# JustinPrivitera/Real_Time_Ray_Tracer

Measured on AMD Instinct MI355X. Metric: Mrays/s + ms/frame at 3840x2160, 16 AO samples, 64 spheres; 1/2/4/8 GPU, higher is better.
Workload: dtype f32

## Files before the change

### include/rt/abi.h

```cpp
#ifndef RT_ABI_H
#define RT_ABI_H

#include <stddef.h>
#include <stdint.h>

#include "layout.h"

#ifdef __cplusplus
extern "C" {
#endif

#define RT_ABI_VERSION 1

enum {
  RT_OK = 0,
  RT_E_INVAL = -1,
  RT_E_NOMEM = -2,
  RT_E_HIP = -3,
  RT_E_NODEV = -4,
  RT_E_STATE = -5
};

enum {
  RT_PROG_AOP_COMPUTE = 1,
// ... 24 lines not shown
int rt_set_stream(rt_ctx* ctx, void* hip_stream);
int rt_use_own_stream(rt_ctx* ctx);
void* rt_get_stream(rt_ctx* ctx);
int rt_enable_pipelining(rt_ctx* ctx, int on, void* output_stream);
void* rt_get_output_stream(rt_ctx* ctx);
void* rt_image_stream(rt_ctx* ctx);
int rt_device_count(void);
int rt_synchronize(rt_ctx* ctx);
int rt_last_hip_error(rt_ctx* ctx);
int rt_debug_fail_next_event_query(rt_ctx* ctx, int hip_error);

int rt_upload_header(rt_ctx* ctx, const void* header, size_t bytes);
int rt_upload_rand_buffer(rt_ctx* ctx, const float* rand_vec4, size_t n_vec4);
int rt_run_program(rt_ctx* ctx, int program, int frame);
int rt_dispatch(rt_ctx* ctx, int mode, int frame);
int rt_compute_frames(rt_ctx* ctx, float* header, int mode, int frame, int n, uint64_t rand_seed,
                      int light_movement);
int rt_set_frame_batch(rt_ctx* ctx, int max_frames);
int rt_set_tile_schedule(rt_ctx* ctx, int on);
int rt_tile_schedule_state(rt_ctx* ctx);
int rt_tile_schedule_orders(rt_ctx* ctx);
int rt_set_cull_cache(rt_ctx* ctx, int on);
int rt_cull_cache_stats(rt_ctx* ctx, long long* fills, long long* cached_launches, size_t* table_bytes);
size_t rt_cull_key(const rt_config* cfg, const void* header, size_t header_bytes, void* key, size_t key_cap);
int rt_download(rt_ctx* ctx, float* pixels, float* normals, float* depth, float* image);
int rt_download_rect(rt_ctx* ctx, int x0, int x1, int y0, int y1, float* pixels, float* normals, float* depth,
                     float* image);
int rt_upload_gbuffer(rt_ctx* ctx, const float* pixels, const float* normals, const float* depth);
void* rt_image_device_ptr(rt_ctx* ctx);
int rt_bind_image(rt_ctx* ctx, void* device_ptr);

int rt_compute_one_shader(rt_ctx* ctx, void* ssbo, int frame_num, int program, float* image);
int rt_compute_two_shaders(rt_ctx* ctx, void* ssbo, int frame_num, int program1, int program2,
                           float* image);

typedef struct rt_group rt_group;
int rt_group_create(int n, const int* devices, const rt_config* cfg, const int* bounds, rt_group** out);
int rt_group_strip_copies(rt_group* g, int i);
int rt_group_force_copies(rt_group* g, int on);
int rt_group_destroy(rt_group* g);
int rt_group_size(rt_group* g);
int rt_group_bounds(rt_group* g, int* bounds);
int rt_group_set_bounds(rt_group* g, const int* bounds);
rt_ctx* rt_group_strip(rt_group* g, int i);
int rt_group_last_hip_error(rt_group* g);
int rt_group_enable_pipelining(rt_group* g, int on);
// ... 67 lines not shown
```

### real_time_ray_tracer_amd/_lib.py

```python
from __future__ import annotations

import ctypes as C
import os
from pathlib import Path

LIB_NAME = "librtrt.so"
LIB_PATH = Path(__file__).resolve().with_name(LIB_NAME)

RT_OK, RT_E_INVAL, RT_E_NOMEM, RT_E_HIP, RT_E_NODEV, RT_E_STATE = 0, -1, -2, -3, -4, -5
RT_PROG_AOP_COMPUTE = 1
RT_PROG_AOP_POSTPROCESSING = 2
RT_PROG_AO_COMPUTE = 3
RT_PROG_P_COMPUTE = 4
RT_PROG_H_COMPUTE = 5
RT_MODE_AO_PP, RT_MODE_AO, RT_MODE_PHONG, RT_MODE_PHONG_REFL = 1, 2, 3, 4
(RT_MATH_SIN, RT_MATH_RANDOM, RT_MATH_SQRT, RT_MATH_DIV, RT_MATH_NORMALIZE, RT_MATH_SPHERE, RT_MATH_SQRT_SWEEP,
 RT_MATH_RCP_SWEEP, RT_MATH_SQRT_TAIL_SWEEP, RT_MATH_SIN_RANGE, RT_MATH_SHADOW,
 RT_MATH_SIN_TABLE) = range(12)
RT_NUM_FRAMES = 8
RT_RECURSION_DEPTH = 20
RT_SHAPE_SPHERE, RT_SHAPE_RECTANGLE, RT_SHAPE_PLANE = 1, 3, 5
HDR_MODE, HDR_HORIZONTAL, HDR_VERTICAL, HDR_LLC, HDR_CAMERA, HDR_LIGHT, HDR_BACKGROUND = range(7)


# ... 10 lines not shown
SIGNATURES = {
    "rt_create": (C.c_int, [C.c_int, C.POINTER(rt_config), C.POINTER(_ctx)]),
    "rt_destroy": (C.c_int, [_ctx]),
    "rt_set_stream": (C.c_int, [_ctx, _vp]),
    "rt_use_own_stream": (C.c_int, [_ctx]),
    "rt_get_stream": (_vp, [_ctx]),
    "rt_enable_pipelining": (C.c_int, [_ctx, C.c_int, _vp]),
    "rt_get_output_stream": (_vp, [_ctx]),
    "rt_image_stream": (_vp, [_ctx]),
    "rt_device_count": (C.c_int, []),
    "rt_synchronize": (C.c_int, [_ctx]),
    "rt_last_hip_error": (C.c_int, [_ctx]),
    "rt_upload_header": (C.c_int, [_ctx, _vp, C.c_size_t]),
    "rt_upload_rand_buffer": (C.c_int, [_ctx, _fp, C.c_size_t]),
    "rt_run_program": (C.c_int, [_ctx, C.c_int, C.c_int]),
    "rt_dispatch": (C.c_int, [_ctx, C.c_int, C.c_int]),
    "rt_compute_frames": (C.c_int, [_ctx, _fp, C.c_int, C.c_int, C.c_int, C.c_uint64, C.c_int]),
    "rt_set_frame_batch": (C.c_int, [_ctx, C.c_int]),
    "rt_set_tile_schedule": (C.c_int, [_ctx, C.c_int]),
    "rt_tile_schedule_state": (C.c_int, [_ctx]),
    "rt_tile_schedule_orders": (C.c_int, [_ctx]),
    "rt_set_cull_cache": (C.c_int, [_ctx, C.c_int]),
    "rt_cull_cache_stats": (C.c_int, [_ctx, C.POINTER(C.c_longlong), C.POINTER(C.c_longlong), C.POINTER(C.c_size_t)]),
    "rt_cull_key": (C.c_size_t, [C.POINTER(rt_config), _vp, C.c_size_t, _vp, C.c_size_t]),
    "rt_download": (C.c_int, [_ctx, _fp, _fp, _fp, _fp]),
    "rt_download_rect": (C.c_int, [_ctx, C.c_int, C.c_int, C.c_int, C.c_int, _fp, _fp, _fp, _fp]),
    "rt_upload_gbuffer": (C.c_int, [_ctx, _fp, _fp, _fp]),
    "rt_image_device_ptr": (_vp, [_ctx]),
    "rt_bind_image": (C.c_int, [_ctx, _vp]),
    "rt_compute_one_shader": (C.c_int, [_ctx, _vp, C.c_int, C.c_int, _fp]),
    "rt_compute_two_shaders": (C.c_int, [_ctx, _vp, C.c_int, C.c_int, C.c_int, _fp]),
    "rt_group_create": (C.c_int, [C.c_int, C.POINTER(C.c_int), C.POINTER(rt_config), C.POINTER(C.c_int),
                                  C.POINTER(_grp)]),
    "rt_group_destroy": (C.c_int, [_grp]),
    "rt_group_size": (C.c_int, [_grp]),
    "rt_group_strip_copies": (C.c_int, [_grp, C.c_int]),
    "rt_group_force_copies": (C.c_int, [_grp, C.c_int]),
    "rt_group_bounds": (C.c_int, [_grp, C.POINTER(C.c_int)]),
    "rt_group_set_bounds": (C.c_int, [_grp, C.POINTER(C.c_int)]),
    "rt_group_strip": (_ctx, [_grp, C.c_int]),
    "rt_group_last_hip_error": (C.c_int, [_grp]),
    "rt_group_enable_pipelining": (C.c_int, [_grp, C.c_int]),
    "rt_group_bind_frame": (C.c_int, [_grp, _vp]),
    "rt_group_frame_device_ptr": (_vp, [_grp]),
    "rt_group_upload_header": (C.c_int, [_grp, _vp, C.c_size_t]),
    "rt_group_dispatch": (C.c_int, [_grp, C.c_int, C.c_int]),
# ... 90 lines not shown
```

### real_time_ray_tracer_amd/csrc/rt_kernels.h

```cpp
#pragma once
#include <hip/hip_runtime.h>

#ifndef RT_NRM_PLANES
#define RT_NRM_PLANES 1
#endif

namespace rt {

constexpr int kMaxFrames = 16;
constexpr int kMaxBatch = 32;
#ifndef RT_HY_BW
#define RT_HY_BW 2
#endif
constexpr int kHyBW = RT_HY_BW, kHyTile = 8 * RT_HY_BW;
constexpr int kCounters = 8;
constexpr int kCounterSlots = 256;

struct FrameParams {
  int W, H;
  int trace_row0, trace_rows;
  int band_row0, band_rows;
  int img_row0, img_rows;
  int nobj;
  int S;
  int spp, D, F, frame;
  int b1_min;
  int pool_rot;
  int tile_run;
  int post_sx, post_sy;
  float inv_spp, fW, fH;
  float inv_W, inv_H;
  float hx, hy, hz;
  float vx, vy, vz;
  float lx, ly, lz;
  float cx, cy, cz;
  float Lx, Ly, Lz;
  float4 bg;
  const float4* shapes;
  const float4* sph;
  const float4* planes;
  int nplanes;
  const float4* clus;
  const unsigned long long* clmask;
  const float4* camrel;
  int ncl;
  const float4* rb;
  float4* out_pix;
  float4* nrm;
  float4* dep;
  const float4* nrm_prev;
  const float4* dep_prev;
  float4* image;
  const float4* raw;
  const float4* hist_pix[kMaxFrames];
  const float4* hist_nrm[kMaxFrames];
  const float4* hist_dep[kMaxFrames];
  unsigned long long* counters;
  unsigned long long* row_counters;
  int mf_n, mf_slot0;
  float4 mf_light[kMaxBatch];
  const float4* mf_rb;
  const unsigned* tile_order;
  unsigned* tile_cost;
  const unsigned long long* cull;
};

constexpr int kAoPool = 256;
constexpr long long ao_pool_count(int trace_rows, int W, int spp) {
  const int TP = kAoPool / spp > 0 ? kAoPool / spp : 1;
  return ((long long)trace_rows * W + TP - 1) / TP;
}

constexpr int kMaxClusters = 64;
constexpr int kClusterWords = 4;

__host__ __device__ constexpr size_t sphere_table(int S) { return (size_t)4 * S; }
__host__ __device__ constexpr size_t plane_table(int S) { return (size_t)5 * S; }
__host__ __device__ constexpr size_t cluster_table(int S) { return (size_t)7 * S; }
__host__ __device__ constexpr size_t cluster_mask_table(int S) { return cluster_table(S) + kMaxClusters; }
__host__ __device__ constexpr size_t camrel_table(int S) {
  return cluster_mask_table(S) + (size_t)(1 + kMaxClusters) * kClusterWords / 2;
}
__host__ __device__ constexpr size_t rand_table(int S) { return camrel_table(S) + (size_t)S; }
__host__ __device__ constexpr size_t table_vec4(int S, int spp) { return rand_table(S) + (size_t)2 * spp; }

enum KernelId { K_AOP = 1, K_POST = 2, K_AO = 3, K_PHONG = 4, K_HYBRID = 5 };

hipError_t launch_program(int program, const FrameParams& p, hipStream_t stream);

hipError_t launch_cull_fill(const FrameParams& p, unsigned long long* table, hipStream_t stream);

struct GbufXfer {
  int W, R, r0, F, kind, to_ref;
  size_t n;
  float4* ref;
  float4* slot[kMaxFrames];
};
hipError_t launch_gbuf_convert(const GbufXfer& x, hipStream_t stream);

hipError_t launch_selftest(int fn, const float* d_in, float* d_out, size_t n, hipStream_t stream);

}
```

### real_time_ray_tracer_amd/csrc/rt_kernels_impl.h

```cpp
#pragma once
#include <hip/hip_runtime.h>

#include "rt_device.h"
#include "rt_kernels.h"

namespace rt {

namespace {

constexpr int kBlock = 256;
constexpr float kGamma = 1.0f / 2.2f;

__device__ __forceinline__ void stage_shapes(const FrameParams& P, float4* lds) {
  const int n = P.nobj;
  for (int k = threadIdx.x; k < 4 * n; k += blockDim.x) {
    int tab = k / n, i = k - tab * n;
    lds[k] = P.shapes[(size_t)tab * P.S + i];
  }
}

__device__ __forceinline__ f3 primary_dir(const FrameParams& P, float hp, float vp) {
  f3 a = mk(P.lx + hp * P.hx, P.ly + hp * P.hy, P.lz + hp * P.hz);
  return normalize(mk(a.x + vp * P.vx, a.y + vp * P.vy, a.z + vp * P.vz));
}
// ... 737 lines not shown

#ifndef RT_AO_MINW
#define RT_AO_MINW 7
#endif
constexpr int kAoMinWaves = RT_AO_MINW;
#ifndef RT_B1_SORT
#define RT_B1_SORT 1
#endif

struct AoConfig {
  static constexpr int SPPC = 0;
  static constexpr int DC = 0;
  static constexpr bool PL = false;
  static constexpr bool CLON = false;
  static constexpr bool CNT = true;
  static constexpr bool MF = false;
  static constexpr bool LAZY = true;
  static constexpr bool TAIL = false;
  static constexpr bool B1 = false;
  static constexpr bool PT = false;
  static constexpr bool PTW = false;
  static constexpr bool SORT = false;
  static constexpr bool CULLC = false;
  static constexpr int ABL = 0;
};
enum : unsigned {
  AO_PL = 1,
  AO_CLON = 2,
  AO_SORT = 4,
  AO_WIDE = 8,
  AO_CNT = 16,
  AO_MF = 32,
  AO_CULLC = 64,
};
template <int SPPC_, int DC_, unsigned FLAGS>
struct AoProd : AoConfig {
  static constexpr int SPPC = SPPC_, DC = DC_;
  static constexpr bool PL = FLAGS & AO_PL, CLON = FLAGS & AO_CLON, SORT = FLAGS & AO_SORT, PTW = FLAGS & AO_WIDE,
                        CNT = FLAGS & AO_CNT, MF = FLAGS & AO_MF, CULLC = FLAGS & AO_CULLC;
  static constexpr bool TAIL = true, B1 = true, PT = true;
};

struct BatchLds {
  int prec, sres, pstop, pkind, perm, order, cmask, rls, geol, total;
};
__host__ __device__ constexpr BatchLds batch_lds_of(int spp, int ntail, bool rls_lds, bool sort) {
  const int TP = kPool / spp > 0 ? kPool / spp : 1, NS = TP * spp;
  BatchLds L{};
  L.prec = 0;
  L.sres = 16 * TP;
  L.pstop = L.sres + 12 * NS;
  L.pkind = L.pstop + 4 * TP;
  L.perm = L.pkind + 4 * ((TP + 1) & ~1);
  L.order = L.perm + 256;
  L.cmask = (L.order + (sort ? kPool : 0) + 7) & ~7;
  L.rls = (L.cmask + 8 * 32 + 15) & ~15;
  L.geol = L.rls + (rls_lds ? 32 * spp : 0);
  L.total = L.geol + 16 * ntail;
  return L;
}
template <class C>
__host__ __device__ constexpr BatchLds batch_lds(int spp, int ntail) {
  return batch_lds_of(spp, ntail, !C::PTW, C::SORT);
}

template <class C>
__global__ __launch_bounds__(64, kAoMinWaves) void ao_batch_kernel(FrameParams P, const float4* __restrict__ geo,
                                                                   const unsigned long long* __restrict__ cullt) {
  constexpr int SPPC = C::SPPC, DC = C::DC, ABL = C::ABL;
  constexpr bool PL = C::PL, CLON = C::CLON, CNT = C::CNT, MF = C::MF, LAZY = C::LAZY, TAIL = C::TAIL, B1 = C::B1,
                 PT = C::PT, PTW = C::PTW, SORT = C::SORT, CULLC = C::CULLC;
  static_assert(!CULLC || !PL, "the cull table holds the spheres' masks only");
  __builtin_amdgcn_s_setprio(1);
  unsigned long long* const cnts = CNT ? P.counters : nullptr;
  unsigned long long* const rowc = CNT ? P.row_counters : nullptr;
  extern __shared__ float4 lds[];
  const int spp = SPPC ? SPPC : P.spp, W = P.W, D = DC ? DC : P.D, nobj = P.nobj;
  const bool use_cl = CLON || P.ncl > 0;
  const int fj = MF ? (int)blockIdx.y : 0;
  const int fslot = MF ? (P.mf_slot0 + fj) % P.F : 0;
  float4* const f_nrm = MF ? (float4*)P.hist_nrm[fslot] : P.nrm;
  float4* const f_dep = MF ? (float4*)P.hist_dep[fslot] : P.dep;
  const float4* const f_nrm_prev = MF ? f_nrm : P.nrm_prev;
  const float4* const f_dep_prev = MF ? f_dep : P.dep_prev;
  float4* const f_out = MF ? (float4*)P.hist_pix[fslot] : P.out_pix;
  float4* const f_img = MF ? (fj == P.mf_n - 1 ? P.image : nullptr) : P.image;
  const float4* const f_rb = MF ? P.mf_rb + (size_t)fj * 2 * spp : P.rb;
  const int TP = kPool / spp > 0 ? kPool / spp : 1;
  const int lane = threadIdx.x;
  const int NS = TP * spp;
  static_assert(!SORT || (LAZY && kPool % 64 == 0 && kPool <= 256), "SORT: hemi is read back from LDS; items are bytes");
  const BatchLds LO = batch_lds<C>(spp, 0);
  char* lbase = (char*)lds;
  float4* prec = (float4*)(lbase + LO.prec);
  float* sres = (float*)(lbase + LO.sres);
// ... 400 lines not shown
        __builtin_amdgcn_s_setprio(0);
        if (ABL == 7) { tsec[4] += 1; tsec[5] += (unsigned long long)__popcll(lm1); }
        if (live) {
          if (PL) plane_pass(P, bpos, bdir, 0.0001f, t, ind);
          ++nseg;
          live = shade(ind, t, bpos, bdir, bhemi, br, bg, bb, D - 1, bitem, false);
        }
        if (ABL == 6) lap(7);
        bdepth = D - 2;
        lap(4);
      }
    }
    unsigned long long lm = __ballot(live);
    if (live) perm[__builtin_amdgcn_mbcnt_hi((unsigned)(lm >> 32), __builtin_amdgcn_mbcnt_lo((unsigned)lm, 0u))] = lane;
    nlive = __popcll(lm);
    cursor = 0;
    next = next + 64 < total ? next + 64 : total;
    __syncthreads();
  };

  if (SORT) {
    constexpr int NC = kPool / 64, NF = 3;
    static_assert(NC * (1 << NF) <= 64, "one cell per lane");
    const int ln = lane_id_here();
    perm[ln] = 0;
    __syncthreads();
    int key[NC];
#pragma unroll
    for (int c = 0; c < NC; ++c) {
      key[c] = 0;
      if (c * 64 < total) {
        const int it = c * 64 + ln;
        f3 h = mk(0.0f, 0.0f, 0.0f);
        if (it < total) {
          const int lp = div_spp(it), aa = it - lp * spp;
          int x, y;
          pool_xy(lp, x, y);
          const float px = (float)x, py = (float)y;
          const float4 f = rbuf[2 * aa], s = rbuf[2 * aa + 1];
          float abe[3];
          grandom_n<3>({f.x + px * s.z, f.z - px * s.z, s.x * px + s.z}, {f.y + py * s.w, f.w - py * s.w, s.y * py + s.w},
                       abe);
          h = normalize(mk(abe[0] * 2.0f - 1.0f, abe[1] * 2.0f - 1.0f, abe[2] * 2.0f - 1.0f));
          sres[it] = h.x;
          sres[NS + it] = h.y;
          sres[2 * NS + it] = h.z;
        }
        const int nv = total - c * 64;
        const unsigned long long mv = nv >= 64 ? ~0ull : (1ull << nv) - 1;
        unsigned own_lo = (unsigned)mv, own_hi = (unsigned)(mv >> 32);
        unsigned oct = 0;
        const float hc[NF] = {h.x, h.y, h.z};
#pragma unroll
        for (int k = NF - 1; k >= 0; --k) {
          const int bits = __float_as_int(hc[k]);
          const unsigned long long m = __ballot(bits < 0);
          const unsigned sgn = (unsigned)(bits >> 31);
          own_lo &= ~((unsigned)m ^ sgn);
          own_hi &= ~((unsigned)(m >> 32) ^ sgn);
          oct = oct << 1 | (unsigned)bits >> 31;
        }
        const int cell = (int)oct * NC + c;
        const int r = (int)__builtin_amdgcn_mbcnt_hi(own_hi, __builtin_amdgcn_mbcnt_lo(own_lo, 0u));
        if (it < total) perm[cell] = __popc(own_lo) + __popc(own_hi);
        key[c] = r | cell << 8;
      }
    }
    __syncthreads();
    {
      const int bin = ln / NC, c = ln % NC;
      const bool in = ln < NC * (1 << NF);
      const int cell = in ? (bin ^ (bin >> 1)) * NC + c : 0;
      const int n = in ? perm[cell] : 0;
      int acc = n;
      acc += __builtin_amdgcn_update_dpp(0, acc, 0x111, 0xf, 0xf, false);
      acc += __builtin_amdgcn_update_dpp(0, acc, 0x112, 0xf, 0xf, false);
      acc += __builtin_amdgcn_update_dpp(0, acc, 0x114, 0xf, 0xf, false);
      acc += __builtin_amdgcn_update_dpp(0, acc, 0x118, 0xf, 0xf, false);
      acc += __builtin_amdgcn_update_dpp(0, acc, 0x142, 0xa, 0xf, false);
      acc += __builtin_amdgcn_update_dpp(0, acc, 0x143, 0xc, 0xf, false);
      __syncthreads();
      if (in) perm[cell] = acc - n;
    }
    __syncthreads();
#pragma unroll
    for (int c = 0; c < NC; ++c) {
      const int it = c * 64 + ln;
      if (it < total) order[perm[key[c] >> 8] + (key[c] & 255)] = (unsigned char)it;
    }
    __syncthreads();
  }

  for (;;) {
    for (;;) {
      unsigned long long need = __ballot(!has);
// ... 508 lines not shown
      out[5 * i] = l.x; out[5 * i + 1] = l.y; out[5 * i + 2] = l.z; out[5 * i + 3] = len;
      out[5 * i + 4] = occ ? 1.0f : 0.0f;
      break;
    }
    case 4: {
      f3 v = normalize(mk(in[3 * i], in[3 * i + 1], in[3 * i + 2]));
      out[3 * i] = v.x; out[3 * i + 1] = v.y; out[3 * i + 2] = v.z;
      break;
    }
    case 5: {
      const float* a = in + 10 * i;
      out[i] = sphere_eval(mk(a[0], a[1], a[2]), mk(a[3], a[4], a[5]), make_float4(a[6], a[7], a[8], a[9]));
      break;
    }
    default: break;
  }
}

size_t shapes_lds_bytes(const FrameParams& p) { return (size_t)4 * p.nobj * sizeof(float4); }
size_t tab_lds_bytes(const FrameParams& p) { return (size_t)5 * (p.nobj > 0 ? p.nobj : 1) * sizeof(float4); }

}

__global__ __launch_bounds__(64) void cull_fill_kernel(FrameParams P, const float4* __restrict__ geo,
                                                       unsigned long long* __restrict__ table) {
  const int spp = P.spp, W = P.W, nobj = P.nobj;
  const int TP = kPool / spp > 0 ? kPool / spp : 1;
  const int lane = threadIdx.x;
  const long long npix = (long long)P.trace_rows * W;
  const unsigned pb = blockIdx.x;
  const long long p0 = (long long)pb * TP;
  const int np = (int)(npix - p0 < TP ? npix - p0 : TP);
  const int yf = P.trace_row0 + (int)(p0 / W), xf = (int)(p0 % W);
  const int yl = P.trace_row0 + (int)((p0 + np - 1) / W), xl = (int)((p0 + np - 1) % W);
  const int nwords = (nobj + 63) >> 6;
  const ConeF cone = pool_cone_f(P, yf == yl ? xf : 0, yf == yl ? xl : W - 1, yf, yl);
  for (int w = 0; w < nwords; ++w) {
    int i = (w << 6) + lane;
    bool keep = i < nobj && !cone_misses_f(cone, geo[i], P.cx, P.cy, P.cz);
    unsigned long long m = __ballot(keep);
    if (lane == 0) table[(size_t)pb * (unsigned)nwords + w] = m;
  }
}

hipError_t launch_cull_fill(const FrameParams& p, unsigned long long* table, hipStream_t stream) {
  const long long pools = ao_pool_count(p.trace_rows, p.W, p.spp);
  if (pools <= 0 || p.nobj <= 0) return hipSuccess;
  hipLaunchKernelGGL(cull_fill_kernel, dim3((unsigned)pools), dim3(64), 0, stream, p, p.shapes + sphere_table(p.S), table);
  return hipGetLastError();
}

constexpr int kRefDepth = 20;
#ifndef RT_B1_SORT_MIN
#define RT_B1_SORT_MIN 48
#endif
constexpr int kB1SortMinObj = RT_B1_SORT_MIN;

struct AoChoice {
  int sppc, dc;
  unsigned flags;
};
constexpr bool operator==(const AoChoice& a, const AoChoice& b) {
  return a.sppc == b.sppc && a.dc == b.dc && a.flags == b.flags;
}
constexpr AoChoice ao_select(int spp, int D, int ncl, int nobj, int nplanes, bool counters, bool multi_frame,
                             bool cull_table) {
  const bool pl = nplanes > 0;
  const bool own = spp == 16 || spp == 4 || (spp == 64 && !pl);
  const bool clon = !pl && (spp == 16 || spp == 64) && D == kRefDepth && ncl > 0;
  return AoChoice{own ? spp : 0, clon ? kRefDepth : 0,
                  (pl ? AO_PL : 0u) | (clon ? AO_CLON : 0u) | (RT_B1_SORT && !pl && nobj >= kB1SortMinObj ? AO_SORT : 0u) |
// ... 10 lines not shown
static_assert(ao_select(16, 20, 9, 65, 0, false, false, false) == AoChoice{16, 20, AO_CLON | kSortBit}, "q");
static_assert(ao_select(16, 20, 0, 10, 1, false, false, false) == AoChoice{16, 0, AO_PL}, "s1");
static_assert(ao_select(4, 20, 0, 10, 1, false, false, false) == AoChoice{4, 0, AO_PL}, "ref");
static_assert(ao_select(16, 20, 8, 64, 0, true, false, false) == AoChoice{16, 20, AO_CLON | kSortBit | AO_CNT}, "counters");
static_assert(ao_select(16, 20, 8, 64, 0, false, true, false) == AoChoice{16, 20, AO_CLON | kSortBit | AO_MF}, "multi-frame");
static_assert(ao_select(16, 20, 8, 64, 0, true, true, false) == AoChoice{16, 20, AO_CLON | kSortBit | AO_MF}, "multi-frame");
static_assert(ao_select(16, 20, 6, kB1SortMinObj - 1, 0, false, false, false) == AoChoice{16, 20, AO_CLON}, "unsorted");
static_assert(ao_select(16, 20, 6, kB1SortMinObj, 0, false, false, false) == AoChoice{16, 20, AO_CLON | kSortBit}, "sorted");
static_assert(ao_select(64, 20, 12, kTailMaxObj, 0, false, false, false) == AoChoice{64, 20, AO_CLON | kSortBit}, "LDS table");
static_assert(ao_select(64, 20, 12, kTailMaxObj + 1, 0, false, false, false) == AoChoice{64, 20, AO_CLON | kSortBit | AO_WIDE}, "wide");
static_assert(ao_select(16, 10, 8, 64, 0, false, false, false) == AoChoice{16, 0, kSortBit}, "depth 10");
static_assert(ao_select(64, 20, 0, 300, 0, false, false, false) == AoChoice{64, 0, kSortBit | AO_WIDE}, "no clusters");
static_assert(ao_select(4, 20, 8, 64, 0, false, false, false) == AoChoice{4, 0, kSortBit}, "spp 4");
static_assert(ao_select(8, 20, 8, 64, 0, true, false, false) == AoChoice{0, 0, kSortBit | AO_CNT}, "spp 8");
static_assert(ao_select(64, 20, 8, 200, 2, false, false, false) == AoChoice{0, 0, AO_PL | AO_WIDE}, "planes, spp 64");
static_assert(ao_select(16, 20, 8, 64, 0, false, false, true) == AoChoice{16, 20, AO_CLON | kSortBit | AO_CULLC}, "c, d cached");
static_assert(ao_select(64, 20, 16, 256, 0, false, false, true) == AoChoice{64, 20, AO_CLON | kSortBit | AO_WIDE | AO_CULLC},
              "e cached");
static_assert(ao_select(16, 20, 8, 64, 0, true, false, true) == AoChoice{16, 20, AO_CLON | kSortBit | AO_CNT | AO_CULLC},
              "counters cached");
static_assert(ao_select(16, 20, 8, 64, 0, false, true, true) == AoChoice{16, 20, AO_CLON | kSortBit | AO_MF | AO_CULLC},
              "multi-frame cached");
static_assert(ao_select(8, 20, 8, 64, 0, false, false, true) == AoChoice{0, 0, kSortBit | AO_CULLC}, "spp 8 cached");
static_assert(ao_select(16, 20, 9, 65, 1, false, false, true) == AoChoice{16, 0, AO_PL}, "p: never cached");
static_assert(ao_select(4, 20, 0, 10, 1, false, false, true) == AoChoice{4, 0, AO_PL}, "ref: never cached");

template <class C>
inline void launch_ao(long long pools, hipStream_t stream, const FrameParams& q) {
  const dim3 g((unsigned)pools, C::MF ? (unsigned)q.mf_n : 1u);
  hipLaunchKernelGGL((ao_batch_kernel<C>), g, dim3(64), (size_t)batch_lds<C>(q.spp, C::PTW ? 64 : q.nobj).total, stream,
                     q, q.sph, q.cull);
}
template <int SPPC, int DC, unsigned SHAPE>
inline void launch_ao_forms(unsigned flags, long long pools, hipStream_t stream, const FrameParams& q) {
  switch (flags & (AO_WIDE | AO_CNT | AO_MF)) {
    case 0: return launch_ao<AoProd<SPPC, DC, SHAPE>>(pools, stream, q);
    case AO_CNT: return launch_ao<AoProd<SPPC, DC, SHAPE | AO_CNT>>(pools, stream, q);
    case AO_MF: return launch_ao<AoProd<SPPC, DC, SHAPE | AO_MF>>(pools, stream, q);
    case AO_WIDE: return launch_ao<AoProd<SPPC, DC, SHAPE | AO_WIDE>>(pools, stream, q);
    case AO_WIDE | AO_CNT: return launch_ao<AoProd<SPPC, DC, SHAPE | AO_WIDE | AO_CNT>>(pools, stream, q);
    case AO_WIDE | AO_MF: return launch_ao<AoProd<SPPC, DC, SHAPE | AO_WIDE | AO_MF>>(pools, stream, q);
  }
}
template <int SPPC, int DC, unsigned SHAPE>
inline void launch_ao_shape(unsigned flags, long long pools, hipStream_t stream, const FrameParams& q) {
  if constexpr (!(SHAPE & AO_PL)) {
// ... 131 lines not shown
```

### real_time_ray_tracer_amd/csrc/rt_shim.hip

```cpp
#include <hip/hip_runtime.h>

#include <algorithm>
#include <chrono>
#include <cmath>
#include <cstdlib>
#include <cstring>
#include <limits>
#include <new>
#include <utility>
#include <vector>

#include "../../include/rt/abi.h"
#include "rt_kernels.h"

namespace {

constexpr int kMaxShapes = 2048;
constexpr int kMaxSpp = 256;
constexpr int kMaxDepth = 65535;
constexpr int kStageSlots = 8;
constexpr int kPipe = 4;
constexpr int kAoStreams = 3;

struct Stage {
// ... 11 lines not shown
  unsigned* h_cost = nullptr;
  unsigned* h_order[2] = {};
  hipStream_t side = nullptr;
  hipEvent_t ev_launch = nullptr, ev_cost = nullptr, ev_order = nullptr;
  hipEvent_t ev_use[2][3] = {};
  hipStream_t used_on[2][3] = {};
  int active = -1;
  int pending = -1;
  bool cost_inflight = false;
  long long launches = 0;
  int orders_taken = 0;
  std::vector<unsigned> cur, next;
};
constexpr int kSchedPeriod = 16;

#ifndef RT_CULL_CACHE_MAX_MB
#define RT_CULL_CACHE_MAX_MB 512
#endif
constexpr size_t kCullCacheMaxBytes = (size_t)RT_CULL_CACHE_MAX_MB << 20;
constexpr int kCullRepeats = 2;
struct CullCache {
  bool on = true;
  bool nomem = false;
  unsigned long long* d_table = nullptr;
  size_t bytes = 0;
  std::vector<unsigned char> key;
  std::vector<unsigned char> next;
  bool have_key = false;
  int repeats = 0;
  bool valid = false;
  hipEvent_t ev_fill = nullptr;
  hipStream_t seen[kAoStreams] = {};
  hipStream_t readers[kAoStreams] = {};
  hipEvent_t ev_read[kAoStreams] = {};
  int n_read = 0;
  long long fills = 0, cached = 0;
};

}

struct rt_ctx {
  int device = 0;
  int inject_query_error = 0;
  rt_config cfg{};
  int own0 = 0, own_rows = 0;
  int band0 = 0, band_rows = 0;
// ... 118 lines not shown
  RT_HIP(c, hipEventRecord(s.done, st));
  s.used = true;
  return RT_OK;
}

void free_sched(TileSched& h) {
  if (h.side) (void)hipStreamSynchronize(h.side);
  if (h.d_cost) (void)hipFree(h.d_cost);
  for (int k = 0; k < 2; ++k) {
    if (h.d_order[k]) (void)hipFree(h.d_order[k]);
    if (h.h_order[k]) (void)hipHostFree(h.h_order[k]);
    for (auto e : h.ev_use[k])
      if (e) (void)hipEventDestroy(e);
  }
  if (h.h_cost) (void)hipHostFree(h.h_cost);
  for (auto e : {h.ev_launch, h.ev_cost, h.ev_order})
    if (e) (void)hipEventDestroy(e);
  if (h.side) (void)hipStreamDestroy(h.side);
  h = TileSched{};
}

void free_all(rt_ctx* c) {
  for (auto& h : c->sched) free_sched(h);
  if (c->cull.d_table) (void)hipFree(c->cull.d_table);
  if (c->cull.ev_fill) (void)hipEventDestroy(c->cull.ev_fill);
  for (auto e : c->cull.ev_read)
    if (e) (void)hipEventDestroy(e);
  for (auto& s : c->stage) {
    if (s.done) (void)hipEventDestroy(s.done);
    if (s.host) (void)hipHostFree(s.host);
  }
  for (int k = 0; k < RT_PROG_COUNT; ++k)
    for (auto& pr : c->pending[k]) {
      (void)hipEventDestroy(pr.e0);
      (void)hipEventDestroy(pr.e1);
    }
  for (auto e : c->event_pool) (void)hipEventDestroy(e);
  for (auto p : c->pix) if (p) (void)hipFree(p);
  for (auto p : c->nrm) if (p) (void)hipFree(p);
  for (auto p : c->dep) if (p) (void)hipFree(p);
  if (c->d_image_own) (void)hipFree(c->d_image_own);
  for (int k = 0; k < kAoStreams; ++k) {
    if (c->d_shapes_buf[k]) (void)hipFree(c->d_shapes_buf[k]);
  }
  if (c->d_counters) (void)hipFree(c->d_counters);
  if (c->d_batch) (void)hipFree(c->d_batch);
  if (c->d_xfer) (void)hipFree(c->d_xfer);
// ... 130 lines not shown

void cull_streams_idle(rt_ctx* c) {
  CullCache& k = c->cull;
  k.n_read = 0;
  for (auto& s : k.readers) s = nullptr;
  for (auto& s : k.seen) s = nullptr;
}

bool cull_note(hipStream_t* set, hipStream_t st) {
  for (int s = 0; s < kAoStreams; ++s) {
    if (set[s] == st) return false;
    if (!set[s]) {
      set[s] = st;
      return true;
    }
  }
  set[0] = st;
  return true;
}

int cull_before(rt_ctx* c, rt::FrameParams& p, hipStream_t st) {
  CullCache& k = c->cull;
  p.cull = nullptr;
  const int nwmax = (c->cfg.num_shapes + 63) / 64;
  const size_t need = (size_t)rt::ao_pool_count(p.trace_rows, p.W, p.spp) * nwmax * sizeof(unsigned long long);
  const bool whole_band = p.trace_row0 == c->band0 && p.trace_rows == c->band_rows;
  if (!k.on || k.nomem || p.nplanes > 0 || p.nobj <= 0 || !whole_band || need == 0 || need > kCullCacheMaxBytes) {
    k.have_key = false;
    return cull_invalidate(c);
  }
  std::vector<unsigned char>& key = k.next;
  key.resize(cull_key(c->cfg, c->header.data(), nullptr, 0));
  if (key.empty() || cull_key(c->cfg, c->header.data(), key.data(), key.size()) != key.size()) {
    k.have_key = false;
    return cull_invalidate(c);
  }
  if (!k.have_key || key != k.key) {
    k.key.swap(key);
    k.have_key = true;
    k.repeats = 0;
    return cull_invalidate(c);
  }
  if (++k.repeats < kCullRepeats) return RT_OK;
  k.repeats = kCullRepeats;
  if (!k.valid) {
    if (!k.d_table) {
      const hipError_t e = hipMalloc(&k.d_table, need);
      if (e != hipSuccess) {
        (void)hipGetLastError();
        k.d_table = nullptr;
        k.nomem = true;
        return RT_OK;
      }
      k.bytes = need;
    }
    if (!k.ev_fill) RT_HIP(c, hipEventCreateWithFlags(&k.ev_fill, hipEventDisableTiming));
    for (int s = 0; s < k.n_read; ++s) RT_HIP(c, hipStreamWaitEvent(st, k.ev_read[s], 0));
    k.n_read = 0;
    const hipError_t e = rt::launch_cull_fill(p, k.d_table, st);
    if (e != hipSuccess) return hip_fail(c, e);
    RT_HIP(c, hipEventRecord(k.ev_fill, st));
    for (auto& s : k.seen) s = nullptr;
    k.seen[0] = st;
    k.valid = true;
    k.fills += 1;
  }
  if (cull_note(k.seen, st)) RT_HIP(c, hipStreamWaitEvent(st, k.ev_fill, 0));
  cull_note(k.readers, st);
  p.cull = k.d_table;
  k.cached += 1;
  return RT_OK;
}

int launch_timed(rt_ctx* c, int program, const rt::FrameParams& p, hipStream_t st) {
  hipEvent_t e0 = nullptr, e1 = nullptr;
  if (c->timing) {
    e0 = get_event(c);
    e1 = get_event(c);
    if (!e0 || !e1) return RT_E_HIP;
    RT_HIP(c, hipEventRecord(e0, st));
  }
  hipError_t e = rt::launch_program(program, p, st);
  if (e != hipSuccess) return hip_fail(c, e);
  if (p.image) c->img_stream = st;
  if (c->timing) {
    RT_HIP(c, hipEventRecord(e1, st));
    c->pending[program].push_back(rt_ctx::Timed{e0, e1, p.mf_n > 0 ? p.mf_n : 1});
  }
  return RT_OK;
}
int launch(rt_ctx* c, int program, const rt::FrameParams& p, hipStream_t st) {
  if (program != RT_PROG_AO_COMPUTE && program != RT_PROG_AOP_COMPUTE) return launch_timed(c, program, p, st);
// ... 832 lines not shown
int rt_tile_schedule_state(rt_ctx* c) {
  if (!c) return RT_E_INVAL;
  if (!c->sched_on) return 0;
  for (auto& h : c->sched)
    if (h.active >= 0) return 2;
  return 1;
}

int rt_tile_schedule_orders(rt_ctx* c) {
  if (!c) return RT_E_INVAL;
  int n = 0;
  for (auto& h : c->sched) n += h.orders_taken;
  return n;
}

int rt_set_cull_cache(rt_ctx* c, int on) {
  if (!c) return RT_E_INVAL;
  RT_HIP(c, hipSetDevice(c->device));
  c->cull.on = on != 0;
  c->cull.have_key = false;
  return cull_invalidate(c);
}

int rt_cull_cache_stats(rt_ctx* c, long long* fills, long long* cached_launches, size_t* table_bytes) {
  if (!c) return RT_E_INVAL;
  if (fills) *fills = c->cull.fills;
  if (cached_launches) *cached_launches = c->cull.cached;
  if (table_bytes) *table_bytes = c->cull.bytes;
  return RT_OK;
}

size_t rt_cull_key(const rt_config* cfg, const void* header, size_t header_bytes, void* key, size_t key_cap) {
  if (!cfg || !header || cfg->width <= 0 || cfg->height <= 0 || cfg->spp <= 0 || cfg->num_shapes < 0 ||
      header_bytes != rt_header_bytes(cfg->num_shapes, cfg->spp))
    return 0;
  rt_config x = *cfg;
  if (x.row_begin == 0 && x.row_end == 0) x.row_end = x.height;
  if (x.row_begin < 0 || x.row_end > x.height || x.row_begin >= x.row_end) return 0;
  return cull_key(x, (const float*)header, (unsigned char*)key, key_cap);
}

int rt_set_frame_batch(rt_ctx* c, int max_frames) {
  if (!c || max_frames < 1) return RT_E_INVAL;
  c->mf_max = std::min(max_frames, rt::kMaxBatch);
  return RT_OK;
}
// ... 260 lines not shown
```

### real_time_ray_tracer_amd/host.py

```python
from __future__ import annotations

import ctypes as C
from dataclasses import dataclass

import numpy as np

from . import _lib
from ._lib import RtError, fptr

AOP_COMPUTE = _lib.RT_PROG_AOP_COMPUTE
AOP_POSTPROCESSING = _lib.RT_PROG_AOP_POSTPROCESSING
AO_COMPUTE = _lib.RT_PROG_AO_COMPUTE
P_COMPUTE = _lib.RT_PROG_P_COMPUTE
H_COMPUTE = _lib.RT_PROG_H_COMPUTE
PROGRAM_NAMES = {AOP_COMPUTE: "aop_compute", AOP_POSTPROCESSING: "aop_postprocessing",
                 AO_COMPUTE: "ao_compute", P_COMPUTE: "p_compute", H_COMPUTE: "h_compute"}

ASPECT_RATIO = 1.333333
FULLSCREEN_ASPECT_RATIO = 1.777777


def header_floats(S: int, AA: int) -> int:
    return 4 * (7 + 5 * S + 2 * AA)

# ... 187 lines not shown
                       light_movement: bool = False) -> int:
        return self._c(self._lib.rt_compute_frames(self.ctx, header._p(), mode, frame, n, rand_seed,
                                                   int(bool(light_movement))), "rt_compute_frames")

    def set_frame_batch(self, max_frames: int):
        self._c(self._lib.rt_set_frame_batch(self.ctx, int(max_frames)), "rt_set_frame_batch")

    def set_tile_schedule(self, on: bool):
        self._c(self._lib.rt_set_tile_schedule(self.ctx, int(bool(on))), "rt_set_tile_schedule")

    def tile_schedule_state(self) -> int:
        return self._c(self._lib.rt_tile_schedule_state(self.ctx), "rt_tile_schedule_state")

    def tile_schedule_orders(self) -> int:
        return self._c(self._lib.rt_tile_schedule_orders(self.ctx), "rt_tile_schedule_orders")

    def set_cull_cache(self, on: bool):
        self._c(self._lib.rt_set_cull_cache(self.ctx, int(bool(on))), "rt_set_cull_cache")

    def cull_cache_stats(self) -> dict:
        f, n, b = C.c_longlong(), C.c_longlong(), C.c_size_t()
        self._c(self._lib.rt_cull_cache_stats(self.ctx, C.byref(f), C.byref(n), C.byref(b)), "rt_cull_cache_stats")
        return {"fills": f.value, "cached_launches": n.value, "table_bytes": b.value}

    def download(self, pixels=True, normals=True, depth=True, image=True) -> GBuffer:
        shp = (self.F, self.W, self.R, 4)
        p = np.empty(shp, np.float32) if pixels else None
        n = np.empty(shp, np.float32) if normals else None
        d = np.empty(shp, np.float32) if depth else None
        im = np.empty((self.R, self.W, 4), np.float32) if image else None
        self._c(self._lib.rt_download(self.ctx, fptr(p), fptr(n), fptr(d), fptr(im)), "rt_download")
        return GBuffer(p, n, d, im)

    def download_rect(self, x0: int, x1: int, y0: int, y1: int, pixels=True, normals=True, depth=True,
                      image=True) -> GBuffer:
        shp = (self.F, x1 - x0, y1 - y0, 4)
        p = np.empty(shp, np.float32) if pixels else None
        n = np.empty(shp, np.float32) if normals else None
        d = np.empty(shp, np.float32) if depth else None
        im = np.empty((y1 - y0, x1 - x0, 4), np.float32) if image else None
        self._c(self._lib.rt_download_rect(self.ctx, x0, x1, y0, y1, fptr(p), fptr(n), fptr(d), fptr(im)),
                "rt_download_rect")
        return GBuffer(p, n, d, im)

    def image(self) -> np.ndarray:
        return self.download(False, False, False, True).image
# ... 254 lines not shown
```

Measured before the change: 66640.

## Sort AO rays by per-pool tangent-frame sectors stored beside cull table

The cached cull-fill kernel now also traces one representative primary ray per pool, builds a tangent frame from the hit normal, and stores two frame axes in a region allocated in front of the cull table. The AO batch kernel, when sorting with the cull cache, bins hemisphere directions into eight sectors of that local frame (sector codes in Gray order) instead of world-axis octants. The intent is more coherent ray bins, since world octants split a hemisphere unevenly, so wavefronts diverge less during traversal. In exchange it adds extra memory, a more expensive fill pass, and two dot products per sample in the sort.

```diff
diff --git a/include/rt/abi.h b/include/rt/abi.h
--- a/include/rt/abi.h
+++ b/include/rt/abi.h
@@ -70,6 +70,8 @@
 int rt_tile_schedule_orders(rt_ctx* ctx);
 int rt_set_cull_cache(rt_ctx* ctx, int on);
 int rt_cull_cache_stats(rt_ctx* ctx, long long* fills, long long* cached_launches, size_t* table_bytes);
+size_t rt_cull_cache_frame_bytes(rt_ctx* ctx);
+int rt_debug_cull_cache_cap(rt_ctx* ctx, size_t bytes);
 size_t rt_cull_key(const rt_config* cfg, const void* header, size_t header_bytes, void* key, size_t key_cap);
 int rt_download(rt_ctx* ctx, float* pixels, float* normals, float* depth, float* image);
 int rt_download_rect(rt_ctx* ctx, int x0, int x1, int y0, int y1, float* pixels, float* normals, float* depth,
diff --git a/real_time_ray_tracer_amd/_lib.py b/real_time_ray_tracer_amd/_lib.py
--- a/real_time_ray_tracer_amd/_lib.py
+++ b/real_time_ray_tracer_amd/_lib.py
@@ -56,6 +56,8 @@
     "rt_tile_schedule_orders": (C.c_int, [_ctx]),
     "rt_set_cull_cache": (C.c_int, [_ctx, C.c_int]),
     "rt_cull_cache_stats": (C.c_int, [_ctx, C.POINTER(C.c_longlong), C.POINTER(C.c_longlong), C.POINTER(C.c_size_t)]),
+    "rt_cull_cache_frame_bytes": (C.c_size_t, [_ctx]),
+    "rt_debug_cull_cache_cap": (C.c_int, [_ctx, C.c_size_t]),
     "rt_cull_key": (C.c_size_t, [C.POINTER(rt_config), _vp, C.c_size_t, _vp, C.c_size_t]),
     "rt_download": (C.c_int, [_ctx, _fp, _fp, _fp, _fp]),
     "rt_download_rect": (C.c_int, [_ctx, C.c_int, C.c_int, C.c_int, C.c_int, _fp, _fp, _fp, _fp]),
diff --git a/real_time_ray_tracer_amd/csrc/rt_kernels.h b/real_time_ray_tracer_amd/csrc/rt_kernels.h
--- a/real_time_ray_tracer_amd/csrc/rt_kernels.h
+++ b/real_time_ray_tracer_amd/csrc/rt_kernels.h
@@ -35,6 +35,7 @@
   float lx, ly, lz;
   float cx, cy, cz;
   float Lx, Ly, Lz;
+  int cull_frames;
   float4 bg;
   const float4* shapes;
   const float4* sph;
@@ -64,6 +65,10 @@
   unsigned* tile_cost;
   const unsigned long long* cull;
 };
+static_assert(offsetof(FrameParams, bg) == 160 && offsetof(FrameParams, cull_frames) == 156,
+              "cull_frames fills the padding in front of bg");
+
+constexpr size_t ao_cull_frame_bytes(long long pools) { return (size_t)pools * 2 * sizeof(float4); }
 
 constexpr int kAoPool = 256;
 constexpr long long ao_pool_count(int trace_rows, int W, int spp) {
@@ -88,7 +93,7 @@
 
 hipError_t launch_program(int program, const FrameParams& p, hipStream_t stream);
 
-hipError_t launch_cull_fill(const FrameParams& p, unsigned long long* table, hipStream_t stream);
+hipError_t launch_cull_fill(const FrameParams& p, unsigned long long* table, bool frames, hipStream_t stream);
 
 struct GbufXfer {
   int W, R, r0, F, kind, to_ref;
diff --git a/real_time_ray_tracer_amd/csrc/rt_kernels_impl.h b/real_time_ray_tracer_amd/csrc/rt_kernels_impl.h
--- a/real_time_ray_tracer_amd/csrc/rt_kernels_impl.h
+++ b/real_time_ray_tracer_amd/csrc/rt_kernels_impl.h
@@ -783,6 +783,7 @@
   static constexpr bool PTW = false;
   static constexpr bool SORT = false;
   static constexpr bool CULLC = false;
+  static constexpr bool NSORT = false;
   static constexpr int ABL = 0;
 };
 enum : unsigned {
@@ -794,11 +795,15 @@
   AO_MF = 32,
   AO_CULLC = 64,
 };
+constexpr bool ao_sorts_by_frame(unsigned flags) {
+  return (flags & (AO_SORT | AO_CULLC | AO_CNT | AO_PL)) == (AO_SORT | AO_CULLC);
+}
 template <int SPPC_, int DC_, unsigned FLAGS>
 struct AoProd : AoConfig {
   static constexpr int SPPC = SPPC_, DC = DC_;
   static constexpr bool PL = FLAGS & AO_PL, CLON = FLAGS & AO_CLON, SORT = FLAGS & AO_SORT, PTW = FLAGS & AO_WIDE,
-                        CNT = FLAGS & AO_CNT, MF = FLAGS & AO_MF, CULLC = FLAGS & AO_CULLC;
+                        CNT = FLAGS & AO_CNT, MF = FLAGS & AO_MF, CULLC = FLAGS & AO_CULLC,
+                        NSORT = ao_sorts_by_frame(FLAGS);
   static constexpr bool TAIL = true, B1 = true, PT = true;
 };
 
@@ -825,6 +830,23 @@
   return batch_lds_of(spp, ntail, !C::PTW, C::SORT);
 }
 
+constexpr int sector_bits(float a, float b) {
+  return (a < 0.0f ? 1 : 0) | (b < 0.0f ? 2 : 0) | ((a < 0.0f ? -a : a) < (b < 0.0f ? -b : b) ? 4 : 0);
+}
+__host__ __device__ constexpr int sector_code(int s) { return (int)(0x26731540u >> (4 * s)) & 7; }
+constexpr bool sector_code_ok() {
+  constexpr float pa[8] = {2, 1, -1, -2, -2, -1, 1, 2}, pb[8] = {1, 2, 2, 1, -1, -2, -2, -1};
+  unsigned seen = 0;
+  for (int s = 0; s < 8; ++s) {
+    if (sector_code(s) != sector_bits(pa[s], pb[s])) return false;
+    const int d = sector_code(s) ^ sector_code((s + 1) & 7);
+    if (d != 1 && d != 2 && d != 4) return false;
+    seen |= 1u << sector_code(s);
+  }
+  return seen == 0xffu;
+}
+static_assert(sector_code_ok(), "sector_code: the 8 sectors in circular order");
+
 template <class C>
 __global__ __launch_bounds__(64, kAoMinWaves) void ao_batch_kernel(FrameParams P, const float4* __restrict__ geo,
                                                                    const unsigned long long* __restrict__ cullt) {
@@ -832,6 +854,8 @@
   constexpr bool PL = C::PL, CLON = C::CLON, CNT = C::CNT, MF = C::MF, LAZY = C::LAZY, TAIL = C::TAIL, B1 = C::B1,
                  PT = C::PT, PTW = C::PTW, SORT = C::SORT, CULLC = C::CULLC;
   static_assert(!CULLC || !PL, "the cull table holds the spheres' masks only");
+  constexpr bool NSORT = C::NSORT;
+  static_assert(!NSORT || (CULLC && SORT), "the sort frames come with the cull table");
   __builtin_amdgcn_s_setprio(1);
   unsigned long long* const cnts = CNT ? P.counters : nullptr;
   unsigned long long* const rowc = CNT ? P.row_counters : nullptr;
@@ -1278,6 +1302,16 @@
   if (SORT) {
     constexpr int NC = kPool / 64, NF = 3;
     static_assert(NC * (1 << NF) <= 64, "one cell per lane");
+    bool framed = false;
+    f3 fe1 = mk(0.0f, 0.0f, 0.0f), fe2 = fe1;
+    if constexpr (NSORT) {
+      framed = P.cull_frames != 0;
+      if (framed) {
+        const float4* const fr = (const float4*)cullt - 2 * ((size_t)pb + 1);
+        fe1 = xyz(fr[0]);
+        fe2 = xyz(fr[1]);
+      }
+    }
     const int ln = lane_id_here();
     perm[ln] = 0;
     __syncthreads();
@@ -1307,14 +1341,27 @@
         unsigned own_lo = (unsigned)mv, own_hi = (unsigned)(mv >> 32);
         unsigned oct = 0;
         const float hc[NF] = {h.x, h.y, h.z};
+        if (NSORT && framed) {
+          const float a = dot(h, fe1), b = dot(h, fe2);
+          const bool sb[NF] = {a < 0.0f, b < 0.0f, fabsf(a) < fabsf(b)};
 #pragma unroll
-        for (int k = NF - 1; k >= 0; --k) {
-          const int bits = __float_as_int(hc[k]);
-          const unsigned long long m = __ballot(bits < 0);
-          const unsigned sgn = (unsigned)(bits >> 31);
-          own_lo &= ~((unsigned)m ^ sgn);
-          own_hi &= ~((unsigned)(m >> 32) ^ sgn);
-          oct = oct << 1 | (unsigned)bits >> 31;
+          for (int k = NF - 1; k >= 0; --k) {
+            const unsigned long long m = __ballot(sb[k]);
+            const unsigned sgn = sb[k] ? ~0u : 0u;
+            own_lo &= ~((unsigned)m ^ sgn);
+            own_hi &= ~((unsigned)(m >> 32) ^ sgn);
+            oct = oct << 1 | (unsigned)sb[k];
+          }
+        } else {
+#pragma unroll
+          for (int k = NF - 1; k >= 0; --k) {
+            const int bits = __float_as_int(hc[k]);
+            const unsigned long long m = __ballot(bits < 0);
+            const unsigned sgn = (unsigned)(bits >> 31);
+            own_lo &= ~((unsigned)m ^ sgn);
+            own_hi &= ~((unsigned)(m >> 32) ^ sgn);
+            oct = oct << 1 | (unsigned)bits >> 31;
+          }
         }
         const int cell = (int)oct * NC + c;
         const int r = (int)__builtin_amdgcn_mbcnt_hi(own_hi, __builtin_amdgcn_mbcnt_lo(own_lo, 0u));
@@ -1326,7 +1373,10 @@
     {
       const int bin = ln / NC, c = ln % NC;
       const bool in = ln < NC * (1 << NF);
-      const int cell = in ? (bin ^ (bin >> 1)) * NC + c : 0;
+      int cell = in ? (bin ^ (bin >> 1)) * NC + c : 0;
+      if constexpr (NSORT) {
+        if (framed) cell = in ? sector_code(bin & 7) * NC + c : 0;
+      }
       const int n = in ? perm[cell] : 0;
       int acc = n;
       acc += __builtin_amdgcn_update_dpp(0, acc, 0x111, 0xf, 0xf, false);
@@ -1881,6 +1931,7 @@
 
 }
 
+template <bool FRAMES>
 __global__ __launch_bounds__(64) void cull_fill_kernel(FrameParams P, const float4* __restrict__ geo,
                                                        unsigned long long* __restrict__ table) {
   const int spp = P.spp, W = P.W, nobj = P.nobj;
@@ -1894,18 +1945,57 @@
   const int yl = P.trace_row0 + (int)((p0 + np - 1) / W), xl = (int)((p0 + np - 1) % W);
   const int nwords = (nobj + 63) >> 6;
   const ConeF cone = pool_cone_f(P, yf == yl ? xf : 0, yf == yl ? xl : W - 1, yf, yl);
+  const f3 cam = mk(P.cx, P.cy, P.cz);
+  f3 dir = cam;
+  if (FRAMES) {
+    int x = xf + np / 2, y = yf;
+    if (x >= W) {
+      const int q = (int)((unsigned)x / (unsigned)W);
+      y += q;
+      x -= q * W;
+    }
+    dir = primary_dir(P, div_rn_by((float)x + 0.0f, P.fW, P.inv_W), div_rn_by((float)y + 0.0f, P.fH, P.inv_H));
+  }
+  float t = -1.0f;
+  int ind = -1;
   for (int w = 0; w < nwords; ++w) {
     int i = (w << 6) + lane;
     bool keep = i < nobj && !cone_misses_f(cone, geo[i], P.cx, P.cy, P.cz);
     unsigned long long m = __ballot(keep);
     if (lane == 0) table[(size_t)pb * (unsigned)nwords + w] = m;
-  }
-}
-
-hipError_t launch_cull_fill(const FrameParams& p, unsigned long long* table, hipStream_t stream) {
+    if (FRAMES) {
+      m = ((unsigned long long)__builtin_amdgcn_readfirstlane((unsigned)(m >> 32)) << 32) |
+          (unsigned)__builtin_amdgcn_readfirstlane((unsigned)m);
+      while (m) {
+        const int j = pop_lowest(m);
+        sphere_candidate(cam, dir, geo[(w << 6) + j], (w << 6) + j, 0.0001f, t, ind);
+      }
+    }
+  }
+  if (FRAMES) {
+    f3 n0 = mk(-dir.x, -dir.y, -dir.z);
+    if (ind >= 0) {
+      const f3 v = (cam + t * dir) - xyz(geo[ind]);
+      n0 = fast_rsq(dot(v, v)) * v;
+    }
+    const bool ry = fabsf(n0.x) >= 0.9f;
+    const f3 c = ry ? mk(-n0.z, 0.0f, n0.x) : mk(0.0f, n0.z, -n0.y);
+    const f3 e1 = fast_rsq(dot(c, c)) * c;
+    const f3 e2 = mk(n0.y * e1.z - n0.z * e1.y, n0.z * e1.x - n0.x * e1.z, n0.x * e1.y - n0.y * e1.x);
+    if (lane == 0) {
+      float4* const fr = (float4*)table - 2 * ((size_t)pb + 1);
+      fr[0] = make_float4(e1.x, e1.y, e1.z, 0.0f);
+      fr[1] = make_float4(e2.x, e2.y, e2.z, 0.0f);
+    }
+  }
+}
+
+hipError_t launch_cull_fill(const FrameParams& p, unsigned long long* table, bool frames, hipStream_t stream) {
   const long long pools = ao_pool_count(p.trace_rows, p.W, p.spp);
   if (pools <= 0 || p.nobj <= 0) return hipSuccess;
-  hipLaunchKernelGGL(cull_fill_kernel, dim3((unsigned)pools), dim3(64), 0, stream, p, p.shapes + sphere_table(p.S), table);
+  const float4* const sph = p.shapes + sphere_table(p.S);
+  if (frames) hipLaunchKernelGGL(cull_fill_kernel<true>, dim3((unsigned)pools), dim3(64), 0, stream, p, sph, table);
+  else hipLaunchKernelGGL(cull_fill_kernel<false>, dim3((unsigned)pools), dim3(64), 0, stream, p, sph, table);
   return hipGetLastError();
 }
 
@@ -1962,6 +2052,13 @@
 static_assert(ao_select(16, 20, 8, 64, 0, false, true, true) == AoChoice{16, 20, AO_CLON | kSortBit | AO_MF | AO_CULLC},
               "multi-frame cached");
 static_assert(ao_select(8, 20, 8, 64, 0, false, false, true) == AoChoice{0, 0, kSortBit | AO_CULLC}, "spp 8 cached");
+static_assert(ao_sorts_by_frame(ao_select(16, 20, 8, 64, 0, false, false, true).flags) == (kSortBit != 0), "c, d cached");
+static_assert(ao_sorts_by_frame(ao_select(64, 20, 16, 256, 0, false, false, true).flags) == (kSortBit != 0), "e cached");
+static_assert(ao_sorts_by_frame(ao_select(16, 20, 8, 64, 0, false, true, true).flags) == (kSortBit != 0), "multi-frame cached");
+static_assert(!ao_sorts_by_frame(ao_select(16, 20, 8, 64, 0, true, false, true).flags), "counters cached: octants");
+static_assert(!ao_sorts_by_frame(ao_select(16, 20, 8, 64, 0, false, false, false).flags), "uncached: octants");
+static_assert(!ao_sorts_by_frame(ao_select(16, 20, 6, kB1SortMinObj - 1, 0, false, false, true).flags), "unsorted");
+static_assert(!ao_sorts_by_frame(ao_select(16, 20, 9, 65, 1, false, false, true).flags), "planes");
 static_assert(ao_select(16, 20, 9, 65, 1, false, false, true) == AoChoice{16, 0, AO_PL}, "p: never cached");
 static_assert(ao_select(4, 20, 0, 10, 1, false, false, true) == AoChoice{4, 0, AO_PL}, "ref: never cached");
 
diff --git a/real_time_ray_tracer_amd/csrc/rt_shim.hip b/real_time_ray_tracer_amd/csrc/rt_shim.hip
--- a/real_time_ray_tracer_amd/csrc/rt_shim.hip
+++ b/real_time_ray_tracer_amd/csrc/rt_shim.hip
@@ -57,6 +57,9 @@
 struct CullCache {
   bool on = true;
   bool nomem = false;
+  size_t cap = kCullCacheMaxBytes;
+  void* d_alloc = nullptr;
+  size_t frame_bytes = 0;
   unsigned long long* d_table = nullptr;
   size_t bytes = 0;
   std::vector<unsigned char> key;
@@ -221,7 +224,7 @@
 
 void free_all(rt_ctx* c) {
   for (auto& h : c->sched) free_sched(h);
-  if (c->cull.d_table) (void)hipFree(c->cull.d_table);
+  if (c->cull.d_alloc) (void)hipFree(c->cull.d_alloc);
   if (c->cull.ev_fill) (void)hipEventDestroy(c->cull.ev_fill);
   for (auto e : c->cull.ev_read)
     if (e) (void)hipEventDestroy(e);
@@ -398,10 +401,11 @@
 int cull_before(rt_ctx* c, rt::FrameParams& p, hipStream_t st) {
   CullCache& k = c->cull;
   p.cull = nullptr;
+  p.cull_frames = 0;
   const int nwmax = (c->cfg.num_shapes + 63) / 64;
   const size_t need = (size_t)rt::ao_pool_count(p.trace_rows, p.W, p.spp) * nwmax * sizeof(unsigned long long);
   const bool whole_band = p.trace_row0 == c->band0 && p.trace_rows == c->band_rows;
-  if (!k.on || k.nomem || p.nplanes > 0 || p.nobj <= 0 || !whole_band || need == 0 || need > kCullCacheMaxBytes) {
+  if (!k.on || k.nomem || p.nplanes > 0 || p.nobj <= 0 || !whole_band || need == 0 || need > k.cap) {
     k.have_key = false;
     return cull_invalidate(c);
   }
@@ -421,19 +425,28 @@
   k.repeats = kCullRepeats;
   if (!k.valid) {
     if (!k.d_table) {
-      const hipError_t e = hipMalloc(&k.d_table, need);
+      size_t fb = rt::ao_cull_frame_bytes(rt::ao_pool_count(p.trace_rows, p.W, p.spp));
+      if (fb > k.cap - need) fb = 0;
+      hipError_t e = hipMalloc(&k.d_alloc, fb + need);
+      if (e != hipSuccess && fb != 0) {
+        (void)hipGetLastError();
+        fb = 0;
+        e = hipMalloc(&k.d_alloc, need);
+      }
       if (e != hipSuccess) {
         (void)hipGetLastError();
-        k.d_table = nullptr;
+        k.d_alloc = nullptr;
         k.nomem = true;
         return RT_OK;
       }
+      k.frame_bytes = fb;
+      k.d_table = (unsigned long long*)((char*)k.d_alloc + fb);
       k.bytes = need;
     }
     if (!k.ev_fill) RT_HIP(c, hipEventCreateWithFlags(&k.ev_fill, hipEventDisableTiming));
     for (int s = 0; s < k.n_read; ++s) RT_HIP(c, hipStreamWaitEvent(st, k.ev_read[s], 0));
     k.n_read = 0;
-    const hipError_t e = rt::launch_cull_fill(p, k.d_table, st);
+    const hipError_t e = rt::launch_cull_fill(p, k.d_table, k.frame_bytes != 0, st);
     if (e != hipSuccess) return hip_fail(c, e);
     RT_HIP(c, hipEventRecord(k.ev_fill, st));
     for (auto& s : k.seen) s = nullptr;
@@ -444,6 +457,7 @@
   if (cull_note(k.seen, st)) RT_HIP(c, hipStreamWaitEvent(st, k.ev_fill, 0));
   cull_note(k.readers, st);
   p.cull = k.d_table;
+  p.cull_frames = k.frame_bytes != 0;
   k.cached += 1;
   return RT_OK;
 }
@@ -1322,6 +1336,15 @@
   return cull_invalidate(c);
 }
 
+int rt_debug_cull_cache_cap(rt_ctx* c, size_t bytes) {
+  if (!c) return RT_E_INVAL;
+  if (c->cull.d_alloc) return RT_E_INVAL;
+  c->cull.cap = bytes && bytes < kCullCacheMaxBytes ? bytes : kCullCacheMaxBytes;
+  return RT_OK;
+}
+
+size_t rt_cull_cache_frame_bytes(rt_ctx* c) { return c ? c->cull.frame_bytes : 0; }
+
 int rt_cull_cache_stats(rt_ctx* c, long long* fills, long long* cached_launches, size_t* table_bytes) {
   if (!c) return RT_E_INVAL;
   if (fills) *fills = c->cull.fills;
diff --git a/real_time_ray_tracer_amd/host.py b/real_time_ray_tracer_amd/host.py
--- a/real_time_ray_tracer_amd/host.py
+++ b/real_time_ray_tracer_amd/host.py
@@ -233,6 +233,12 @@
         f, n, b = C.c_longlong(), C.c_longlong(), C.c_size_t()
         self._c(self._lib.rt_cull_cache_stats(self.ctx, C.byref(f), C.byref(n), C.byref(b)), "rt_cull_cache_stats")
         return {"fills": f.value, "cached_launches": n.value, "table_bytes": b.value}
+
+    def cull_cache_frame_bytes(self) -> int:
+        return int(self._lib.rt_cull_cache_frame_bytes(self.ctx))
+
+    def debug_cull_cache_cap(self, nbytes: int):
+        self._c(self._lib.rt_debug_cull_cache_cap(self.ctx, int(nbytes)), "rt_debug_cull_cache_cap")
 
     def download(self, pixels=True, normals=True, depth=True, image=True) -> GBuffer:
         shp = (self.F, self.W, self.R, 4)
```

Result: faster. 68150, median of 6 (+2.3%).
